# ade-ma/LibRedio

Measured on AMD Instinct MI355X. Metric: MSamples/s through FIR+FFT+resample chain, higher is better.
Workload: dtype f32

## Files before the change

libredio_amd/csrc/chain_v4.hip:

```cpp
#ifndef REDIO_EXP_CHAIN_NT
#define REDIO_EXP_CHAIN_NT 3
#endif
#include "fir_core.h"
#include "fft_wave.h"
#include "redio_internal.h"
#include "../../include/redio.h"
#include <type_traits>

namespace redio {

typedef float v4f_t __attribute__((ext_vector_type(4)));

template <int N, typename F>
__device__ __forceinline__ void static_for4(F &&f)
{
    if constexpr (N > 0) {
        static_for4<N - 1>(f);
        f(std::integral_constant<int, N - 1>{});
    }
}

template <int K, int D, bool FUSED, int WPS, int CH, bool FIR_ONLY, bool TWP, bool IN_U8, bool PF2, bool RES, int SCH>
__device__ __forceinline__ void chain_v4_body(const float2 *__restrict__ x, const float *__restrict__ taps,
                                              const float2 *__restrict__ tw, float2 *__restrict__ out,
                                              long nblocks, long blocks_per_wave, long wave, unsigned long long *dbg, long dbg_cap)
{
    unsigned long long t0c = 0, t0r = 0;
    if (dbg) { t0c = __builtin_amdgcn_s_memtime(); t0r = __builtin_amdgcn_s_memrealtime(); }
    constexpr int R = 4;
    using G = FirGeomV<K, D, R>;
    constexpr int SUB_OUT = 64 * R;
    constexpr int SUB_NEW = SUB_OUT * D;
    constexpr int HALO = G::tile_in(SUB_OUT) - SUB_NEW;
    static_assert(HALO % 2 == 0 && SUB_NEW % 128 == 0 && 4 * SUB_OUT == 1024, "geometry");
    constexpr int HALO_V = HALO / 2;
    constexpr int NLD = SUB_NEW / 2 / 64;
    static_assert(HALO_V <= 64, "the halo moves with one instruction per lane");
    extern __shared__ __attribute__((aligned(16))) char smem[];
    v4f_t *xs4 = reinterpret_cast<v4f_t *>(smem);
    float2 *ex = reinterpret_cast<float2 *>(smem);

    const int lane = threadIdx.x;
    const long b0 = wave * blocks_per_wave;
    if (b0 >= nblocks) return;
    const long b1 = (b0 + blocks_per_wave < nblocks) ? b0 + blocks_per_wave : nblocks;
    const long nsub = 4 * (b1 - b0);
    typename std::conditional<RES, FirTapsResident<K>, FirNoResidentTaps>::type rtaps;
    if constexpr (RES) fir_taps_resident_load(rtaps, taps);
    using pair_t = typename std::conditional<IN_U8, unsigned, v4f_t>::type;
    const pair_t *src0 = (IN_U8 ? reinterpret_cast<const pair_t *>(reinterpret_cast<const unsigned *>(x) + b0 * 512 * (long)D)
                                : reinterpret_cast<const pair_t *>(x + b0 * 1024 * (long)D)) + lane;
    auto samples = [](pair_t w) -> v4f_t {
        if constexpr (IN_U8) return v4f_t{i2f(w & 255u), i2f((w >> 8) & 255u), i2f((w >> 16) & 255u), i2f(w >> 24)};
        else return w;
    };

    pair_t pre[NLD], pre2[PF2 ? NLD : 1];
    __amdgpu_buffer_rsrc_t rs;
    if constexpr (PF2) {
        static_assert(!PF2 || !IN_U8, "PF2: cf32 input");
        rs = __builtin_amdgcn_make_buffer_rsrc(const_cast<float2 *>(x + b0 * 1024 * (long)D), 0, (int)((HALO + nsub * SUB_NEW) * 8), 0x00020000);
    }
    auto fetch_to = [&](pair_t(&dst)[NLD], long j) {
        if constexpr (PF2) {
            typedef unsigned v4u_t __attribute__((ext_vector_type(4)));
            const unsigned vo = 16u * (unsigned)lane + (unsigned)((HALO + j * SUB_NEW) * 8);
            static_for4<NLD>([&](auto I) {
                constexpr int k = I.value;
                const v4u_t w = __builtin_amdgcn_raw_buffer_load_b128(rs, vo + 1024u * (k & 3), 4096 * (k >> 2), 2 );
                dst[k] = __builtin_bit_cast(v4f_t, w);
            });
        } else {
            const pair_t *src = src0 + HALO_V + j * (SUB_NEW / 2);
#if REDIO_EXP_CHAIN_NT & 1
            static_for4<NLD>([&](auto I) { dst[I.value] = __builtin_nontemporal_load(src + 64 * I.value); });
#else
            static_for4<NLD>([&](auto I) { dst[I.value] = src[64 * I.value]; });
#endif
        }
    };
    auto park_from = [&](pair_t(&from)[NLD]) {
#if REDIO_EXP_ABLATE == 3
#pragma unroll
        for (int i = 0; i < NLD; ++i) { pair_t keep = from[i]; asm volatile("" : : "v"(keep)); }
#else
        static_for4<NLD>([&](auto I) { xs4[G::lds_index(HALO + 2 * (lane + 64 * I.value)) / 2] = samples(from[I.value]); });
#endif
    };

    if (lane < HALO_V) xs4[G::lds_index(2 * lane) / 2] = samples(src0[0]);
    static_assert(SCH == 0 || (!PF2 && !FIR_ONLY && TWP && WPS == 2), "the block schedules: the transforming product forms");
    constexpr int EXH_OFF = G::lds_elems(SUB_OUT) > FFT1KN_LDS ? G::lds_elems(SUB_OUT) : FFT1KN_LDS;
    constexpr int T12_OFF = EXH_OFF + (SCH == 2 ? FFT1KN_HALF_LDS : 0);
    static_assert(SCH == 0 || (T12_OFF + 60) * sizeof(float2) <= 160 * 1024 / 8 - 480, "within the request of chain_v4_lds at two waves per SIMD");
    if constexpr ((PF2 || SCH != 0) && !FIR_ONLY) {
        if (lane < 60) {
            const int k4 = lane / 15, i = lane % 15;
            const int idx = i < 3 ? 64 * k4 * (i + 1) : 16 * (k4 + 4 * ((i - 3) / 3)) * ((i - 3) % 3 + 1);
            ex[T12_OFF + lane] = tw[idx];
        }
    }
    fetch_to(pre, 0);
    park_from(pre);
    wave_lds_fence();

    float2 a[16];
#pragma unroll
    for (int i = 0; i < 16; ++i) a[i] = make_float2(0.f, 0.f);
    Fft1knTw34 t34;
    if (!FIR_ONLY && TWP) fft1kn_load_tw34(t34, lane, tw);
    auto step = [&](long j, auto ahead, auto place, pair_t(&req)[NLD], pair_t(&parked)[NLD]) {
        constexpr int AHEAD = decltype(ahead)::value, S = decltype(place)::value;
        const bool more = S >= 0 || j + 1 < nsub;
        if (S >= 0 || j + AHEAD < nsub) fetch_to(req, j + AHEAD);
        float2 acc[R];
#pragma unroll
        for (int r = 0; r < R; ++r) acc[r] = make_float2(0.f, 0.f);
        int lf = lane;
        asm volatile("" : "+v"(lf));
        if constexpr (RES) fir_lane_v_res<K, D, R, FUSED, CH>(xs4, lf, rtaps, acc);
        else fir_lane_v<K, D, R, FUSED, CH>(xs4, lf, taps, acc);
        if (FIR_ONLY) {
            v4f_t *y4 = reinterpret_cast<v4f_t *>(out + (b0 * 4 + j) * SUB_OUT) + 2 * lane;
            y4[0] = v4f_t{acc[0].x, acc[0].y, acc[1].x, acc[1].y};
            y4[1] = v4f_t{acc[2].x, acc[2].y, acc[3].x, acc[3].y};
        } else {
#pragma unroll
            for (int i = 0; i < 12; ++i) a[i] = a[i + 4];
#pragma unroll
            for (int r = 0; r < R; ++r) a[12 + r] = acc[r];
        }
        wave_lds_fence();
        v4f_t halo = v4f_t{0.f, 0.f, 0.f, 0.f};
        if (more && lf < HALO_V) halo = xs4[G::lds_index(SUB_NEW + 2 * lf) / 2];
        if (!FIR_ONLY && (S == 3 || (S < 0 && (j & 3) == 3))) {
            wave_lds_fence();
            int ln = lane;
            asm volatile("" : "+v"(ln));
            Fft1knTw12 t12;
            if constexpr (PF2) {
                const float2 *T = ex + T12_OFF + 15 * (ln >> 4);
#pragma unroll
                for (int i = 0; i < 3; ++i) t12.a[i] = T[i];
#pragma unroll
                for (int i = 0; i < 12; ++i) t12.b[i] = T[3 + i];
            } else fft1kn_load_tw12(t12, ln, tw);
            if (!TWP) fft1kn_load_tw34(t34, ln, tw);
            fft1kn_wave_tw<false>(a, ex, tw, t12, t34, out + (b0 + (j >> 2)) * 1024, ln);
            wave_lds_fence();
        }
        if (more) {
            if (lf < HALO_V) xs4[G::lds_index(2 * lf) / 2] = halo;
            park_from(parked);
        }
        wave_lds_fence();
    };
    [[maybe_unused]] float2 one = make_float2(0.f, 0.f);
    if constexpr (SCH != 0) {
        one = tw[0];
        asm volatile("" : "+v"(one.x), "+v"(one.y));
    }
    [[maybe_unused]] auto t12_lds = [&](Fft1knTw12 &t12, int ln) {
        const float2 *T = ex + T12_OFF + 15 * (ln >> 4);
#pragma unroll
        for (int i = 0; i < 3; ++i) t12.a[i] = T[i];
#pragma unroll
        for (int i = 0; i < 12; ++i) t12.b[i] = T[3 + i];
    };
    [[maybe_unused]] auto sstep = [&](long j, auto place, bool more_, bool xform_, auto &&hook) {
        constexpr int S = decltype(place)::value;
        const bool more = S < 3 || more_, xform = S == 3 && xform_;
        if (more) fetch_to(pre, j + 1);
        float2 acc[R];
#pragma unroll
        for (int r = 0; r < R; ++r) acc[r] = make_float2(0.f, 0.f);
        int lf = lane;
        asm volatile("" : "+v"(lf));
        if constexpr (RES) fir_lane_v_res<K, D, R, FUSED, CH>(xs4, lf, rtaps, acc, hook);
        else fir_lane_v<K, D, R, FUSED, CH>(xs4, lf, taps, acc, hook);
#pragma unroll
        for (int r = 0; r < R; ++r) a[4 * S + r] = acc[r];
        wave_lds_fence();
        v4f_t halo = v4f_t{0.f, 0.f, 0.f, 0.f};
        if (more && lf < HALO_V) halo = xs4[G::lds_index(SUB_NEW + 2 * lf) / 2];
        if (xform) {
            wave_lds_fence();
            int ln = lane;
            asm volatile("" : "+v"(ln));
            Fft1knTw12 t12;
            t12_lds(t12, ln);
            const float2 one1[1] = {one};
            fft1kn_wave_tw<false>(a, ex, one1, t12, t34, out + (b0 + (j >> 2)) * 1024, ln);
            wave_lds_fence();
        }
        if (more) {
            if (lf < HALO_V) xs4[G::lds_index(2 * lf) / 2] = halo;
            park_from(pre);
        }
        wave_lds_fence();
    };
    using S0 = std::integral_constant<int, 0>;
    using S1 = std::integral_constant<int, 1>;
    using S2 = std::integral_constant<int, 2>;
    using S3 = std::integral_constant<int, 3>;
    if constexpr (SCH == 1) {
        const long nb = b1 - b0;
#pragma unroll 1
        for (long blk = 0; blk < nb; ++blk) {
            sstep(4 * blk, S0{}, true, false, FirNoHook{});
            sstep(4 * blk + 1, S1{}, true, false, FirNoHook{});
            sstep(4 * blk + 2, S2{}, true, false, FirNoHook{});
            sstep(4 * blk + 3, S3{}, blk + 1 < nb, true, FirNoHook{});
        }
    } else if constexpr (SCH == 2) {
        constexpr int NCH = fir_num_chunks<K, D, R, CH>();
        const long nb = b1 - b0;
        sstep(0, S0{}, true, false, FirNoHook{});
#pragma unroll 1
        for (long blk = 0;; ++blk) {
            sstep(4 * blk + 1, S1{}, true, false, FirNoHook{});
            sstep(4 * blk + 2, S2{}, true, false, FirNoHook{});
            const bool more = blk + 1 < nb;
            sstep(4 * blk + 3, S3{}, more, !more, FirNoHook{});
            if (!more) break;
            float2 ap[16], u[16];
#pragma unroll
            for (int i = 0; i < 16; ++i) ap[i] = a[i];
            int ln = lane;
            asm volatile("" : "+v"(ln));
            Fft1knTw12 t12;
            float2 *dst = out + (b0 + blk) * 1024;
            auto piece = [&](auto C) {
                fft1kn_wave_piece<decltype(C)::value, false>(ap, u, ex + EXH_OFF, one, ex + T12_OFF + 15 * (ln >> 4), t12, t34, dst, ln);
            };
            sstep(4 * blk + 4, S0{}, true, false, piece);
            if constexpr (NCH < FFT1KN_PIECES)
                static_for4<FFT1KN_PIECES - NCH>([&](auto I) { piece(std::integral_constant<int, NCH + I.value>{}); });
        }
    } else if constexpr (PF2) {
        fetch_to(pre, 1);
        using two = std::integral_constant<int, 2>;
#pragma unroll 1
        for (long j = 0; j < nsub; j += 4) {
            step(j, two{}, std::integral_constant<int, 0>{}, pre2, pre);
            step(j + 1, two{}, std::integral_constant<int, 1>{}, pre, pre2);
            step(j + 2, two{}, std::integral_constant<int, 2>{}, pre2, pre);
            step(j + 3, two{}, std::integral_constant<int, 3>{}, pre, pre2);
        }
    } else {
#pragma unroll 1
        for (long j = 0; j < nsub; ++j) step(j, std::integral_constant<int, 1>{}, std::integral_constant<int, -1>{}, pre, pre);
    }
    if (dbg && lane == 0 && (long)blockIdx.x < dbg_cap) {
        dbg[4 * blockIdx.x] = __builtin_amdgcn_s_memtime() - t0c;
        dbg[4 * blockIdx.x + 1] = __builtin_amdgcn_s_memrealtime() - t0r;
        dbg[4 * blockIdx.x + 2] = t0r;
        unsigned xcc = 0;
        asm volatile("s_getreg_b32 %0, hwreg(HW_REG_XCC_ID)" : "=s"(xcc));
        unsigned hwid = 0;
        asm volatile("s_getreg_b32 %0, hwreg(HW_REG_HW_ID)" : "=s"(hwid));
        dbg[4 * blockIdx.x + 3] = ((unsigned long long)xcc << 32) | hwid;
    }
}

template <int WPS, bool FIR_ONLY, bool TWP, bool PF2, bool RES>
constexpr int chain_v4_sched()
{
    return (WPS == 2 && !FIR_ONLY && TWP && !PF2) ? 1 : 0;
}

template <int K, int D, bool FUSED, int WPS, int CH, bool FIR_ONLY = false, bool TWP = false, bool IN_U8 = false, bool PF2 = false>
__global__ __launch_bounds__(64, WPS) void chain_v4_kernel(const float2 *__restrict__ x, const float *__restrict__ taps,
                                                           const float2 *__restrict__ tw, float2 *__restrict__ out,
                                                           long nblocks, long blocks_per_wave, unsigned long long *dbg, long dbg_cap)
{
    chain_v4_body<K, D, FUSED, WPS, CH, FIR_ONLY, TWP, IN_U8, PF2, true, chain_v4_sched<WPS, FIR_ONLY, TWP, PF2, true>()>(x, taps, tw, out, nblocks, blocks_per_wave, (long)blockIdx.x, dbg, dbg_cap);
}
template <int K, int D, bool FUSED, int WPS, int CH, bool FIR_ONLY = false, bool TWP = false, bool IN_U8 = false, bool PF2 = false>
__global__ __launch_bounds__(64, WPS) void chain_v4_anytaps_kernel(const float2 *__restrict__ x, const float *__restrict__ taps,
                                                                   const float2 *__restrict__ tw, float2 *__restrict__ out,
                                                                   long nblocks, long blocks_per_wave, unsigned long long *dbg, long dbg_cap)
{
    chain_v4_body<K, D, FUSED, WPS, CH, FIR_ONLY, TWP, IN_U8, PF2, false, chain_v4_sched<WPS, FIR_ONLY, TWP, PF2, false>()>(x, taps, tw, out, nblocks, blocks_per_wave, (long)blockIdx.x, dbg, dbg_cap);
}

#ifdef REDIO_MEASURE
template <int K, int D, bool FUSED>
__global__ __launch_bounds__(64, 2) void chain_v4_sched2_kernel(const float2 *__restrict__ x, const float *__restrict__ taps,
                                                                const float2 *__restrict__ tw, float2 *__restrict__ out,
                                                                long nblocks, long blocks_per_wave, unsigned long long *dbg, long dbg_cap)
{
    chain_v4_body<K, D, FUSED, 2, 8, false, true, false, false, true, 2>(x, taps, tw, out, nblocks, blocks_per_wave, (long)blockIdx.x, dbg, dbg_cap);
}
#endif

struct ChainList {
    const float2 *x[REDIO_LIST_MAX];
    float2 *out[REDIO_LIST_MAX];
    long nblocks[REDIO_LIST_MAX];
    unsigned wave0[REDIO_LIST_MAX + 1];
    int count;
};

template <int K, int D, bool FUSED, bool RES>
__device__ __forceinline__ void chain_v4_list_body(const ChainList &list, const float *__restrict__ taps, const float2 *__restrict__ tw,
                                                   long blocks_per_wave)
{
    const unsigned w = blockIdx.x;
    int m = 0;
    for (int i = 1; i < list.count; ++i) m = w >= list.wave0[i] ? i : m;
    m = __builtin_amdgcn_readfirstlane(m);
    chain_v4_body<K, D, FUSED, 2, 8, false, true, false, false, RES, chain_v4_sched<2, false, true, false, RES>()>(list.x[m], taps, tw, list.out[m], list.nblocks[m], blocks_per_wave,
                                                                     (long)(w - list.wave0[m]), nullptr, 0);
}

template <int K, int D, bool FUSED>
__global__ __launch_bounds__(64, 2) void chain_v4_list_kernel(const ChainList list, const float *__restrict__ taps,
                                                              const float2 *__restrict__ tw, long blocks_per_wave)
{
    chain_v4_list_body<K, D, FUSED, true>(list, taps, tw, blocks_per_wave);
}
template <int K, int D, bool FUSED>
__global__ __launch_bounds__(64, 2) void chain_v4_anytaps_list_kernel(const ChainList list, const float *__restrict__ taps,
                                                                      const float2 *__restrict__ tw, long blocks_per_wave)
{
    chain_v4_list_body<K, D, FUSED, false>(list, taps, tw, blocks_per_wave);
}

long chain_v4_blocks_per_wave(long nblocks, int WPS)
{
    long waves = 4L * WPS * num_cus();
    if (waves > nblocks) waves = nblocks;
    if (waves < 1) waves = 1;
    long bpw = nblocks / (6 * waves);
    if (bpw < 1) bpw = 1;
    if (bpw > 4) bpw = 4;
    if (const char *e = measure_env("REDIO_CHAIN_BPW")) { const long v = atol(e); if (v >= 1) bpw = v; }
    return bpw;
}

template <int K, int D, int WPS, bool PF2 = false>
static constexpr size_t chain_v4_lds()
{
    static_assert(WPS == 2 || WPS == 3, "two wavefronts per SIMD (the chain: its transform needs 197 registers) or three (the FIR alone: 94-145)");
    using G = FirGeomV<K, D, 4>;
    constexpr int ELEMS = (G::lds_elems(256) > FFT1KN_LDS ? G::lds_elems(256) : FFT1KN_LDS) + (PF2 ? 64 : 0);
    constexpr size_t LDS_NEED = (size_t)ELEMS * sizeof(float2);
    static_assert(4 * WPS * LDS_NEED <= 160 * 1024, "4*WPS waves per CU");
    constexpr size_t LDS = (160 * 1024 / (4 * WPS)) - 480 > LDS_NEED ? (160 * 1024 / (4 * WPS)) - 480 : LDS_NEED;
    static_assert((4 * WPS + 1) * LDS > 160 * 1024, "one more wave must not fit");
    return LDS;
}

template <int K, int D, int WPS, int CH, bool FIR_ONLY = false, bool TWP = false, bool IN_U8 = false, bool PF2 = false>
static hipError_t launch_v4_t(const float2 *x, const float *taps, bool pal, const float2 *tw, float2 *out, long nblocks, bool fused,
                              hipStream_t s, unsigned long long *dbg, long dbg_cap = 0)
{
    constexpr size_t LDS = chain_v4_lds<K, D, WPS, PF2>();
    const long bpw = chain_v4_blocks_per_wave(nblocks, WPS);
    const long grid = (nblocks + bpw - 1) / bpw;
    if (pal) {
        if (fused) hipLaunchKernelGGL((chain_v4_kernel<K, D, true, WPS, CH, FIR_ONLY, TWP, IN_U8, PF2>), dim3((unsigned)grid), dim3(64), LDS, s, x, taps, tw, out, nblocks, bpw, dbg, dbg_cap);
        else hipLaunchKernelGGL((chain_v4_kernel<K, D, false, WPS, CH, FIR_ONLY, TWP, IN_U8, PF2>), dim3((unsigned)grid), dim3(64), LDS, s, x, taps, tw, out, nblocks, bpw, dbg, dbg_cap);
    } else {
        if (fused) hipLaunchKernelGGL((chain_v4_anytaps_kernel<K, D, true, WPS, CH, FIR_ONLY, TWP, IN_U8, PF2>), dim3((unsigned)grid), dim3(64), LDS, s, x, taps, tw, out, nblocks, bpw, dbg, dbg_cap);
        else hipLaunchKernelGGL((chain_v4_anytaps_kernel<K, D, false, WPS, CH, FIR_ONLY, TWP, IN_U8, PF2>), dim3((unsigned)grid), dim3(64), LDS, s, x, taps, tw, out, nblocks, bpw, dbg, dbg_cap);
    }
    return hipGetLastError();
// ... 106 lines not shown
```

libredio_amd/csrc/fft_wave.h:

```cpp
#pragma once
#include "fft_core.h"

namespace redio {

__device__ __forceinline__ void wave_lds_fence()
{
    __builtin_amdgcn_fence(__ATOMIC_RELEASE, "wavefront");
    __builtin_amdgcn_wave_barrier();
    __builtin_amdgcn_fence(__ATOMIC_ACQUIRE, "wavefront");
}

template <bool INV, typename TwPtr>
__device__ __forceinline__ void fft1k_wave_stages0to3(float2 (&v)[16], float2 *ex, TwPtr tw, const Fft1kTw &t, int lane)
{
    fft1k_passA<INV>(v, tw);
    wave_lds_fence();
#pragma unroll
    for (int k4 = 0; k4 < 4; ++k4)
#pragma unroll
        for (int k3 = 0; k3 < 4; ++k3) ex[fft1k_A_store(lane, k3, k4)] = v[k3 + 4 * k4];
    wave_lds_fence();
#pragma unroll
    for (int e = 0; e < 16; ++e) v[e] = ex[fft1k_B_load(lane, e)];
    wave_lds_fence();
    fft1k_passB<INV>(v, t);
#pragma unroll
    for (int k2 = 0; k2 < 4; ++k2)
#pragma unroll
        for (int k1 = 0; k1 < 4; ++k1) ex[fft1k_B_store(lane, k1, k2)] = v[k1 + 4 * k2];
    wave_lds_fence();
#pragma unroll
    for (int q = 0; q < 4; ++q)
#pragma unroll
        for (int j = 0; j < 4; ++j) v[4 * q + j] = ex[fft1k_C_load(lane, q, j)];
}

template <bool INV, typename DstPtr, typename TwPtr>
__device__ __forceinline__ void fft1k_wave_regs(float2 (&v)[16], DstPtr dst, float2 *ex, TwPtr tw, const Fft1kTw &t, int lane)
{
    fft1k_wave_stages0to3<INV>(v, ex, tw, t, lane);
    fft1k_passC<INV>(v, t);
#pragma unroll
    for (int q = 0; q < 4; ++q)
#pragma unroll
        for (int j = 0; j < 4; ++j) dst[lane + 64 * q + 256 * j] = v[4 * q + j];
}

template <bool INV, typename SrcPtr>
__device__ __forceinline__ void fft1k_wave(SrcPtr src, float2 *dst, float2 *ex,
                                           const float2 *__restrict__ tw, int lane)
{
    float2 v[16];
#pragma unroll
    for (int t = 0; t < 16; ++t) v[t] = src[lane + 64 * t];
    Fft1kTw t;
    fft1k_load_tw(t, lane, tw);
    fft1k_wave_regs<INV>(v, dst, ex, tw, t, lane);
}

}

namespace redio {

__device__ __forceinline__ void fft1kn_store_spectrum(const float2 (&a)[16], float2 *dst, int ln)
{
#pragma unroll
    for (int k0 = 0; k0 < 4; ++k0)
#pragma unroll
#if defined(REDIO_EXP_CHAIN_NT) && (REDIO_EXP_CHAIN_NT & 2)
        for (int k1 = 0; k1 < 4; ++k1) {
            typedef float nt_v2f __attribute__((ext_vector_type(2)));
            __builtin_nontemporal_store(nt_v2f{a[k1 + 4 * k0].x, a[k1 + 4 * k0].y}, reinterpret_cast<nt_v2f *>(dst + ln + 64 * k1 + 256 * k0));
        }
#else
        for (int k1 = 0; k1 < 4; ++k1) dst[ln + 64 * k1 + 256 * k0] = a[k1 + 4 * k0];
#endif
}

template <bool INV>
__device__ __forceinline__ void fft1kn_wave_tw(float2 (&a)[16], float2 *ex, const float2 *__restrict__ tw, const Fft1knTw12 &t12,
                                               const Fft1knTw34 &t34, float2 *dst, int ln)
{
    fft1kn_stage0<INV>(a, tw);
#pragma unroll
    for (int k4 = 0; k4 < 4; ++k4)
#pragma unroll
        for (int d0 = 0; d0 < 4; ++d0) ex[fft1kn_x1_store(ln, k4, d0)] = a[4 * k4 + d0];
    wave_lds_fence();
#pragma unroll
    for (int e = 0; e < 16; ++e) a[e] = ex[fft1kn_x1_load(ln, e)];
    wave_lds_fence();
    fft1kn_pass12<INV>(a, t12);
#pragma unroll
    for (int k3 = 0; k3 < 4; ++k3)
#pragma unroll
        for (int k2 = 0; k2 < 4; ++k2) ex[fft1kn_x2_store(ln, k2, k3)] = a[k2 + 4 * k3];
    wave_lds_fence();
#pragma unroll
    for (int f = 0; f < 16; ++f) a[f] = ex[fft1kn_x2_load(ln, f)];
    wave_lds_fence();
    fft1kn_pass34<INV>(a, t34);
    fft1kn_store_spectrum(a, dst, ln);
}

constexpr int FFT1KN_PIECES = 8;
template <int P, bool INV>
__device__ __forceinline__ void fft1kn_wave_piece(float2 (&a)[16], float2 (&u)[16], float2 *exh, float2 one, const float2 *T12, Fft1knTw12 &t12,
                                                  const Fft1knTw34 &t34, float2 *dst, int ln)
{
    if constexpr (P == 0) {
        const float2 one1[1] = {one};
        fft1kn_stage0<INV>(a, one1);
        if (fft1kn_x1h_store_half(ln) == 0) {
#pragma unroll
            for (int k4 = 0; k4 < 4; ++k4)
#pragma unroll
                for (int d0 = 0; d0 < 4; ++d0) exh[fft1kn_x1h_store(ln, k4, d0)] = a[4 * k4 + d0];
        }
    } else if constexpr (P == 1 || P == 2) {
        constexpr int h = P - 1;
        wave_lds_fence();
#pragma unroll
        for (int e = 8 * h; e < 8 * h + 8; ++e) u[e] = exh[fft1kn_x1h_load(ln, e)];
        wave_lds_fence();
        if constexpr (h == 0) {
            if (fft1kn_x1h_store_half(ln) == 1) {
#pragma unroll
                for (int k4 = 0; k4 < 4; ++k4)
#pragma unroll
                    for (int d0 = 0; d0 < 4; ++d0) exh[fft1kn_x1h_store(ln, k4, d0)] = a[4 * k4 + d0];
            }
        } else {
#pragma unroll
            for (int i = 0; i < 3; ++i) t12.a[i] = T12[i];
#pragma unroll
            for (int i = 0; i < 12; ++i) t12.b[i] = T12[3 + i];
        }
    } else if constexpr (P == 3) {
        fft1kn_pass12<INV>(u, t12);
        if (fft1kn_x2h_store_half(ln) == 0) {
#pragma unroll
            for (int k3 = 0; k3 < 4; ++k3)
#pragma unroll
                for (int k2 = 0; k2 < 4; ++k2) exh[fft1kn_x2h_store(ln, k2, k3)] = u[k2 + 4 * k3];
        }
    } else if constexpr (P == 4 || P == 5) {
        constexpr int h = P - 4;
        wave_lds_fence();
#pragma unroll
        for (int f = 0; f < 16; ++f)
            if (fft1kn_x2h_load_half(f) == h) a[f] = exh[fft1kn_x2h_load(ln, f)];
        wave_lds_fence();
        if constexpr (h == 0) {
            if (fft1kn_x2h_store_half(ln) == 1) {
#pragma unroll
                for (int k3 = 0; k3 < 4; ++k3)
#pragma unroll
                    for (int k2 = 0; k2 < 4; ++k2) exh[fft1kn_x2h_store(ln, k2, k3)] = u[k2 + 4 * k3];
            }
        }
    } else if constexpr (P == 6) {
        fft1kn_pass34<INV>(a, t34);
    } else if constexpr (P == 7) {
        fft1kn_store_spectrum(a, dst, ln);
    }
}

template <bool INV>
__device__ __forceinline__ void fft1kn_wave(float2 (&a)[16], float2 *ex, const float2 *__restrict__ tw, float2 *dst, int ln)
{
    Fft1knTw12 t12;
    Fft1knTw34 t34;
    fft1kn_load_tw12(t12, ln, tw);
    fft1kn_load_tw34(t34, ln, tw);
    fft1kn_wave_tw<INV>(a, ex, tw, t12, t34, dst, ln);
}

}
```

libredio_amd/csrc/fir_core.h:

```cpp
#pragma once
#include "redio_device.h"
#ifndef REDIO_EXP_ABLATE
#define REDIO_EXP_ABLATE 0
#endif
#include <type_traits>

namespace redio {

template <int K, int D, int R>
struct FirGeom {
    static constexpr int LSTR = R * D;
    static constexpr int SPAN = (R - 1) * D + K;
    static constexpr bool PAD = (LSTR % 2) == 0;
    RD_HD static constexpr int lds_index(int n) { return PAD ? n + n / LSTR : n; }
    RD_HD static constexpr int tile_in(int tile_out) { return (tile_out - 1) * D + K; }
    RD_HD static constexpr int lds_elems(int tile_out) { return lds_index(tile_in(tile_out) - 1) + 1; }
};

template <typename T, int K, int D, int R, bool FUSED, typename LdsPtr, typename TapPtr>
RD_HD void fir_lane(LdsPtr xs, int lane_slot, TapPtr h, T (&acc)[R])
{
    using G = FirGeom<K, D, R>;
    const int base = lane_slot * (G::LSTR + (G::PAD ? 1 : 0));
#pragma unroll
    for (int m = 0; m < G::SPAN; ++m) {
        const T xv = xs[base + G::lds_index(m)];
#pragma unroll
        for (int r = 0; r < R; ++r) {
            const int j = m - r * D;
            if (j >= 0 && j < K) acc[r] = mac<FUSED>(xv, h[j], acc[r]);
        }
    }
}

}

namespace redio {

template <int K, int D, int R>
struct FirGeomV {
    static constexpr int LSTR = R * D;
    static_assert(LSTR % 2 == 0, "16-byte windows need an even lane stride");
    static constexpr int SPAN = (R - 1) * D + K;
    static constexpr int PADN = ((LSTR / 2) % 2 == 1) ? 0 : 2;
    static constexpr int LANE_STRIDE = LSTR + PADN;
    RD_HD static constexpr int lds_index(int n) { return n + PADN * (n / LSTR); }
    RD_HD static constexpr int tile_in(int tile_out) { return (tile_out - 1) * D + K; }
    RD_HD static constexpr int lds_elems(int tile_out) { return (lds_index(tile_in(tile_out) - 1) + 2) & ~1; }
};

template <int N, typename F>
RD_HD void fir_static_for(F &&f)
{
    if constexpr (N > 0) {
        fir_static_for<N - 1>(f);
        f(std::integral_constant<int, N - 1>{});
    }
}

template <int K, int D, int R, int CH>
struct FirChunkTaps {
    static constexpr int NT = 2 * CH + (R - 1) * D;
    RD_HD static constexpr int lo(int c) { return 2 * CH * c - (R - 1) * D; }
};

struct FirNoHook {
    template <typename C>
    RD_HD void operator()(C) const {}
};
template <int K, int D, int R, int CH>
RD_HD constexpr int fir_num_chunks() { return ((FirGeomV<K, D, R>::SPAN + 1) / 2 + CH - 1) / CH; }

template <int c, int K, int D, int R, bool FUSED, int CH, typename Q, typename Lds4Ptr, typename TapPtr, typename Hook>
RD_HD void fir_chunks_v(Lds4Ptr xs4, int base4, TapPtr h, Q (&q)[2][CH],
                        float (&hb)[2][FirChunkTaps<K, D, R, CH>::NT], float2 (&acc)[R], Hook &hook)
{
    using G = FirGeomV<K, D, R>;
    using T = FirChunkTaps<K, D, R, CH>;
    constexpr int NRD = (G::SPAN + 1) / 2;
    constexpr int NCH = (NRD + CH - 1) / CH;
    if constexpr (c < NCH) {
        RD_PIN_SV(hb[c & 1][T::NT - 1], q[c & 1][0]);
        fir_static_for<CH>([&](auto I) {
            constexpr int i = (c + 1) * CH + I.value;
#if REDIO_EXP_ABLATE == 1
            if constexpr (i < NRD && (I.value & 1)) q[(c + 1) & 1][I.value] = q[(c + 1) & 1][I.value - 1];
            else
#endif
            if constexpr (i < NRD) q[(c + 1) & 1][I.value] = xs4[base4 + G::lds_index(2 * i) / 2];
        });
        fir_static_for<T::NT>([&](auto J) {
            constexpr int j = T::lo(c + 1) + J.value;
            if constexpr (c + 1 < NCH && j >= 0 && j < K) hb[(c + 1) & 1][J.value] = h[j];
        });
        hook(std::integral_constant<int, c>{});
        fir_static_for<CH>([&](auto I) {
            constexpr int m = 2 * (c * CH + I.value);
            if constexpr (m < G::SPAN) {
                const Q v = q[c & 1][I.value];
                const float2 x0 = make_float2(v.x, v.y), x1 = make_float2(v.z, v.w);
                fir_static_for<R>([&](auto RR) {
                    constexpr int r = RR.value;
#if REDIO_EXP_ABLATE == 2
                    if constexpr (r & 1) return;
#endif
                    constexpr int j0 = m - r * D, j1 = m + 1 - r * D;
                    if constexpr (j0 >= 0 && j0 < K) acc[r] = mac<FUSED>(x0, hb[c & 1][j0 - T::lo(c)], acc[r]);
                    if constexpr (j1 >= 0 && j1 < K && m + 1 < G::SPAN) acc[r] = mac<FUSED>(x1, hb[c & 1][j1 - T::lo(c)], acc[r]);
                });
            }
        });
#pragma unroll
        for (int r = 0; r < R; ++r) RD_PIN_F2(acc[r]);
        RD_SCHED_BARRIER();
        fir_chunks_v<c + 1, K, D, R, FUSED, CH>(xs4, base4, h, q, hb, acc, hook);
    }
}

template <int K, int D, int R, bool FUSED, int CH = 8 , typename Lds4Ptr, typename TapPtr, typename Hook>
RD_HD void fir_lane_v(Lds4Ptr xs4, int lane_slot, TapPtr h, float2 (&acc)[R], Hook &&hook)
{
    using G = FirGeomV<K, D, R>;
    using Q = typename std::remove_cv<typename std::remove_reference<decltype(xs4[0])>::type>::type;
    constexpr int NRD = (G::SPAN + 1) / 2;
    using T = FirChunkTaps<K, D, R, CH>;
    const int base4 = lane_slot * (G::LANE_STRIDE / 2);
    Q q[2][CH];
    float hb[2][T::NT];
    fir_static_for<T::NT>([&](auto J) {
        constexpr int j = T::lo(0) + J.value;
        hb[0][J.value] = (j >= 0 && j < K) ? h[j] : 0.0f;
        hb[1][J.value] = 0.0f;
    });
    fir_static_for<CH>([&](auto I) {
        constexpr int i = I.value;
        if constexpr (i < NRD) q[0][i] = xs4[base4 + G::lds_index(2 * i) / 2];
    });
    fir_chunks_v<0, K, D, R, FUSED, CH>(xs4, base4, h, q, hb, acc, hook);
}
template <int K, int D, int R, bool FUSED, int CH = 8, typename Lds4Ptr, typename TapPtr>
RD_HD void fir_lane_v(Lds4Ptr xs4, int lane_slot, TapPtr h, float2 (&acc)[R])
{
    fir_lane_v<K, D, R, FUSED, CH>(xs4, lane_slot, h, acc, FirNoHook{});
}

template <int K>
struct FirTapsResident {
    static constexpr int NE = (K + 1) / 2;
    static constexpr int NP = (NE + 1) / 2;
    static_assert(K >= 3, "a pair never reads past the taps");
    RD_HD static constexpr int elem(int j) { return j < K - 1 - j ? j : K - 1 - j; }
    unsigned long long p[NP];
};

struct FirNoResidentTaps {};

template <int K, typename TapPtr>
RD_HD void fir_taps_resident_load(FirTapsResident<K> &t, TapPtr h)
{
    fir_static_for<FirTapsResident<K>::NP>([&](auto I) {
        constexpr int i = I.value;
#if defined(__HIP_DEVICE_COMPILE__)
        typedef unsigned long long u64a __attribute__((may_alias));
        t.p[i] = reinterpret_cast<const u64a *>(&h[0])[i];
        asm volatile("" : "+s"(t.p[i]));
#else
        unsigned lo, hi;
        const float a = h[2 * i], b = h[2 * i + 1];
        __builtin_memcpy(&lo, &a, 4);
        __builtin_memcpy(&hi, &b, 4);
        t.p[i] = (unsigned long long)lo | ((unsigned long long)hi << 32);
#endif
    });
}

template <int K, int D, int R>
struct FirLive {
    RD_HD static constexpr int lo(int m) { return m - (K - 1) <= 0 ? 0 : (m - (K - 1) + D - 1) / D; }
    RD_HD static constexpr int hi(int m) { return m / D < R - 1 ? m / D : R - 1; }
};

#if defined(__HIP_DEVICE_COMPILE__)
typedef redio_v2f fir_acc_t;
#else
typedef float2 fir_acc_t;
#endif

template <int m0, int K, int D, int R, bool TWO >
struct FirReadPlan {
    using L = FirLive<K, D, R>;
    using T = FirTapsResident<K>;
#if REDIO_EXP_ABLATE == 2
    RD_HD static constexpr bool live(int k) { return !(k & 1) && (k < 4 || TWO) && (k & 3) >= L::lo(m0 + k / 4) && (k & 3) <= L::hi(m0 + k / 4) && (k & 3) < R; }
#else
    RD_HD static constexpr bool live(int k) { return (k < 4 || TWO) && (k & 3) >= L::lo(m0 + k / 4) && (k & 3) <= L::hi(m0 + k / 4) && (k & 3) < R; }
#endif
    RD_HD static constexpr int elem(int k) { return live(k) ? T::elem(m0 + k / 4 - (k & 3) * D) : 0; }
    RD_HD static constexpr int pair(int k) { return elem(k) / 2; }
    RD_HD static constexpr unsigned en() { unsigned v = 0; for (int k = 0; k < 8; ++k) v |= (live(k) ? 1u : 0u) << k; return v; }
    RD_HD static constexpr unsigned hi() { unsigned v = 0; for (int k = 0; k < 8; ++k) v |= (unsigned)(elem(k) & 1) << k; return v; }
    RD_HD static constexpr unsigned nop_fused()
    {
        unsigned v = 0;
        int prev = m0 == 0 ? 0 : L::hi(m0 - 1);
        for (int k = 0; k < 8; ++k)
            if (live(k)) { if ((k & 3) == prev) v |= 1u << k; prev = k & 3; }
        return v;
    }
    RD_HD static constexpr unsigned nop_exact()
    {
        unsigned v = 0;
        for (int i = 0; i < 2; ++i) {
            int n = 0;
            for (int r = 0; r < 4; ++r) n += live(4 * i + r) ? 1 : 0;
            if (n == 1) v |= 1u << i;
        }
        return v;
    }
};

#if defined(__HIP_DEVICE_COMPILE__)
#define RD_FMA_SLOT(k, r, i)                                                                                             \
    ".if (%[nb] >> " #k ") & 1\ns_nop 0\n.endif\n"                                                                      \
    ".if (%[en] >> " #k ") & 1\n.if (%[hi] >> " #k ") & 1\n"                                                            \
    "v_pk_fma_f32 %[a" #r "], %[x" #i "], %[t" #k "], %[a" #r "] op_sel:[0,1,0] op_sel_hi:[1,1,1]\n.else\n"               \
    "v_pk_fma_f32 %[a" #r "], %[x" #i "], %[t" #k "], %[a" #r "] op_sel:[0,0,0] op_sel_hi:[1,0,1]\n.endif\n.endif\n"
#define RD_MUL_SLOT(k, r, i)                                                                                             \
    ".if (%[en] >> " #k ") & 1\n.if (%[hi] >> " #k ") & 1\n"                                                            \
    "v_pk_mul_f32 %[d" #r "], %[x" #i "], %[t" #k "] op_sel:[0,1] op_sel_hi:[1,1]\n.else\n"                               \
    "v_pk_mul_f32 %[d" #r "], %[x" #i "], %[t" #k "] op_sel:[0,0] op_sel_hi:[1,0]\n.endif\n.endif\n"
#define RD_ADD_SLOT(k, r) ".if (%[en] >> " #k ") & 1\nv_pk_add_f32 %[a" #r "], %[a" #r "], %[d" #r "]\n.endif\n"
#define RD_ONE_NOP(i) ".if (%[nb] >> " #i ") & 1\ns_nop 0\n.endif\n"
template <int m0, int K, int D, int R, bool FUSED, bool TWO>
RD_D void fir_read_res(redio_v2f x0, redio_v2f x1, const FirTapsResident<K> &t, redio_v2f (&a)[R])
{
    static_assert(R == 4, "four accumulators per lane");
    using P = FirReadPlan<m0, K, D, R, TWO>;
    if constexpr (FUSED)
        asm volatile(RD_FMA_SLOT(0, 0, 0) RD_FMA_SLOT(1, 1, 0) RD_FMA_SLOT(2, 2, 0) RD_FMA_SLOT(3, 3, 0)
                     RD_FMA_SLOT(4, 0, 1) RD_FMA_SLOT(5, 1, 1) RD_FMA_SLOT(6, 2, 1) RD_FMA_SLOT(7, 3, 1)
                     : [a0] "+v"(a[0]), [a1] "+v"(a[1]), [a2] "+v"(a[2]), [a3] "+v"(a[3])
                     : [x0] "v"(x0), [x1] "v"(x1), [t0] "s"(t.p[P::pair(0)]), [t1] "s"(t.p[P::pair(1)]), [t2] "s"(t.p[P::pair(2)]),
                       [t3] "s"(t.p[P::pair(3)]), [t4] "s"(t.p[P::pair(4)]), [t5] "s"(t.p[P::pair(5)]), [t6] "s"(t.p[P::pair(6)]),
                       [t7] "s"(t.p[P::pair(7)]), [en] "i"(P::en()), [hi] "i"(P::hi()), [nb] "i"(P::nop_fused()));
    else {
        redio_v2f d0, d1, d2, d3;
        asm volatile(RD_MUL_SLOT(0, 0, 0) RD_MUL_SLOT(1, 1, 0) RD_MUL_SLOT(2, 2, 0) RD_MUL_SLOT(3, 3, 0) RD_ONE_NOP(0)
                     RD_ADD_SLOT(0, 0) RD_ADD_SLOT(1, 1) RD_ADD_SLOT(2, 2) RD_ADD_SLOT(3, 3)
                     RD_MUL_SLOT(4, 0, 1) RD_MUL_SLOT(5, 1, 1) RD_MUL_SLOT(6, 2, 1) RD_MUL_SLOT(7, 3, 1) RD_ONE_NOP(1)
                     RD_ADD_SLOT(4, 0) RD_ADD_SLOT(5, 1) RD_ADD_SLOT(6, 2) RD_ADD_SLOT(7, 3)
                     : [a0] "+v"(a[0]), [a1] "+v"(a[1]), [a2] "+v"(a[2]), [a3] "+v"(a[3]), [d0] "=&v"(d0), [d1] "=&v"(d1), [d2] "=&v"(d2),
                       [d3] "=&v"(d3)
                     : [x0] "v"(x0), [x1] "v"(x1), [t0] "s"(t.p[P::pair(0)]), [t1] "s"(t.p[P::pair(1)]), [t2] "s"(t.p[P::pair(2)]),
                       [t3] "s"(t.p[P::pair(3)]), [t4] "s"(t.p[P::pair(4)]), [t5] "s"(t.p[P::pair(5)]), [t6] "s"(t.p[P::pair(6)]),
                       [t7] "s"(t.p[P::pair(7)]), [en] "i"(P::en()), [hi] "i"(P::hi()), [nb] "i"(P::nop_exact()));
    }
}
#undef RD_FMA_SLOT
#undef RD_MUL_SLOT
#undef RD_ADD_SLOT
#undef RD_ONE_NOP
#else
template <int m0, int K, int D, int R, bool FUSED, bool TWO>
RD_HD void fir_read_res(float2 x0, float2 x1, const FirTapsResident<K> &t, float2 (&a)[R])
{
    using P = FirReadPlan<m0, K, D, R, TWO>;
    for (int k = 0; k < 8; ++k) {
        if (!P::live(k)) continue;
        const int el = P::elem(k);
        const unsigned w = (unsigned)(t.p[el / 2] >> (32 * (el & 1)));
        float h;
        __builtin_memcpy(&h, &w, 4);
        a[k & 3] = mac<FUSED>(k < 4 ? x0 : x1, h, a[k & 3]);
    }
}
#endif

template <int c, int K, int D, int R, bool FUSED, int CH, typename Q, typename Lds4Ptr, typename Hook>
RD_HD void fir_chunks_res(Lds4Ptr xs4, int base4, const FirTapsResident<K> &t, Q (&q)[2][CH], fir_acc_t (&acc)[R], Hook &hook)
{
    using G = FirGeomV<K, D, R>;
    constexpr int NRD = (G::SPAN + 1) / 2;
    constexpr int NCH = (NRD + CH - 1) / CH;
    if constexpr (c < NCH) {
        RD_PIN_V(q[c & 1][0]);
        fir_static_for<CH>([&](auto I) {
            constexpr int i = (c + 1) * CH + I.value;
#if REDIO_EXP_ABLATE == 1
            if constexpr (i < NRD && (I.value & 1)) q[(c + 1) & 1][I.value] = q[(c + 1) & 1][I.value - 1];
            else
#endif
            if constexpr (i < NRD) q[(c + 1) & 1][I.value] = xs4[base4 + G::lds_index(2 * i) / 2];
        });
        hook(std::integral_constant<int, c>{});
        fir_static_for<CH>([&](auto I) {
            constexpr int m = 2 * (c * CH + I.value);
            if constexpr (m < G::SPAN) {
                const Q v = q[c & 1][I.value];
#if defined(__HIP_DEVICE_COMPILE__)
                const fir_acc_t x0 = __builtin_shufflevector(v, v, 0, 1), x1 = __builtin_shufflevector(v, v, 2, 3);
#else
                const fir_acc_t x0 = make_float2(v.x, v.y), x1 = make_float2(v.z, v.w);
#endif
                fir_read_res<m, K, D, R, FUSED, (m + 1 < G::SPAN)>(x0, x1, t, acc);
            }
        });
        RD_SCHED_BARRIER();
        fir_chunks_res<c + 1, K, D, R, FUSED, CH>(xs4, base4, t, q, acc, hook);
    }
}

template <int K, int D, int R, bool FUSED, int CH = 8, typename Lds4Ptr, typename Hook>
RD_HD void fir_lane_v_res(Lds4Ptr xs4, int lane_slot, const FirTapsResident<K> &t, float2 (&acc)[R], Hook &&hook)
{
    using G = FirGeomV<K, D, R>;
    using Q = typename std::remove_cv<typename std::remove_reference<decltype(xs4[0])>::type>::type;
    constexpr int NRD = (G::SPAN + 1) / 2;
    const int base4 = lane_slot * (G::LANE_STRIDE / 2);
    Q q[2][CH];
    fir_static_for<CH>([&](auto I) {
        constexpr int i = I.value;
        if constexpr (i < NRD) q[0][i] = xs4[base4 + G::lds_index(2 * i) / 2];
    });
    fir_acc_t a[R];
#if defined(__HIP_DEVICE_COMPILE__)
#pragma unroll
// ... 57 lines not shown
```

Baseline: 529,700.

## Use buffer loads/stores, hoist LDS slot indices, and overlap prologue loads

Adds a REDIO_EXP_SEAM switch, defaulting to all options on. It routes input fetches and spectrum/FIR output stores through buffer resources with scalar offsets and nontemporal policy bits. LDS park and halo slot indices are hoisted out of the loop, and the halo read moves into the last FIR chunk hook. The prologue issues all global loads (halo head, first tile, twiddles, resident taps) before any LDS writes, so the latencies overlap. This aims to cut address arithmetic and serialized prologue latency, at the cost of more live registers and sched_barriers that constrain the compiler's scheduling.

```diff
diff --git a/libredio_amd/csrc/chain_v4.hip b/libredio_amd/csrc/chain_v4.hip
--- a/libredio_amd/csrc/chain_v4.hip
+++ b/libredio_amd/csrc/chain_v4.hip
@@ -1,5 +1,8 @@
 #ifndef REDIO_EXP_CHAIN_NT
 #define REDIO_EXP_CHAIN_NT 3
+#endif
+#ifndef REDIO_EXP_SEAM
+#define REDIO_EXP_SEAM 15
 #endif
 #include "fir_core.h"
 #include "fft_wave.h"
@@ -10,6 +13,8 @@
 namespace redio {
 
 typedef float v4f_t __attribute__((ext_vector_type(4)));
+
+constexpr int chain_gcd(int a, int b) { return b == 0 ? a : chain_gcd(b, a % b); }
 
 template <int N, typename F>
 __device__ __forceinline__ void static_for4(F &&f)
@@ -48,27 +53,57 @@
     typename std::conditional<RES, FirTapsResident<K>, FirNoResidentTaps>::type rtaps;
     if constexpr (RES) fir_taps_resident_load(rtaps, taps);
     using pair_t = typename std::conditional<IN_U8, unsigned, v4f_t>::type;
-    const pair_t *src0 = (IN_U8 ? reinterpret_cast<const pair_t *>(reinterpret_cast<const unsigned *>(x) + b0 * 512 * (long)D)
+    [[maybe_unused]] const pair_t *src0 = (IN_U8 ? reinterpret_cast<const pair_t *>(reinterpret_cast<const unsigned *>(x) + b0 * 512 * (long)D)
                                 : reinterpret_cast<const pair_t *>(x + b0 * 1024 * (long)D)) + lane;
     auto samples = [](pair_t w) -> v4f_t {
         if constexpr (IN_U8) return v4f_t{i2f(w & 255u), i2f((w >> 8) & 255u), i2f((w >> 16) & 255u), i2f(w >> 24)};
         else return w;
     };
 
+    constexpr bool HOIST = (REDIO_EXP_SEAM & 1) != 0, BUF = PF2 || (REDIO_EXP_SEAM & 2) != 0, EARLY = (REDIO_EXP_SEAM & 4) != 0,
+                   PRO = (REDIO_EXP_SEAM & 8) != 0;
+    auto slot = [](int p) { return G::lds_index(2 * p) / 2; };
+    constexpr int HSTR = G::LSTR / 2;
+    static_assert((SUB_NEW / 2) % HSTR == 0, "a sub-tile is a whole number of lane strides");
+    constexpr int HALO_DELTA = G::lds_index(SUB_NEW) / 2;
+    constexpr int PER0 = G::PADN == 0 ? 1 : HSTR / chain_gcd(64, HSTR), PER = PER0 < NLD ? PER0 : NLD;
+    constexpr int PARK_STEP = G::lds_index(2 * 64 * PER) / 2;
+    static_assert(PER == NLD || (64 * PER) % HSTR == 0, "park slots repeat with period PER");
+    auto halo_slots = [&](int lf, int &src, int &dst) {
+        dst = slot(lf);
+        if constexpr (EARLY) src = dst + (lf < HALO_V ? HALO_DELTA : 0);
+        else src = slot(SUB_NEW / 2 + lf);
+    };
+    [[maybe_unused]] int park4[PER], hsrc4 = 0, hdst4 = 0;
+    if constexpr (HOIST) {
+        static_for4<PER>([&](auto I) { park4[I.value] = slot(HALO_V + lane + 64 * I.value); });
+        halo_slots(lane, hsrc4, hdst4);
+    }
+
     pair_t pre[NLD], pre2[PF2 ? NLD : 1];
-    __amdgpu_buffer_rsrc_t rs;
-    if constexpr (PF2) {
+    constexpr unsigned PB = sizeof(pair_t);
+    constexpr int NT_LD = (REDIO_EXP_CHAIN_NT & 1) ? 2 : 0, NT_ST = (REDIO_EXP_CHAIN_NT & 2) ? 2 : 0;
+    typedef unsigned v4u_t __attribute__((ext_vector_type(4)));
+    typedef unsigned v2u_t __attribute__((ext_vector_type(2)));
+    [[maybe_unused]] __amdgpu_buffer_rsrc_t ri, ro;
+    if constexpr (BUF) {
         static_assert(!PF2 || !IN_U8, "PF2: cf32 input");
-        rs = __builtin_amdgcn_make_buffer_rsrc(const_cast<float2 *>(x + b0 * 1024 * (long)D), 0, (int)((HALO + nsub * SUB_NEW) * 8), 0x00020000);
-    }
+        const char *xb = reinterpret_cast<const char *>(x) + b0 * (512 * (long)D) * PB;
+        ri = __builtin_amdgcn_make_buffer_rsrc(const_cast<char *>(xb), 0, (int)((HALO_V + nsub * (SUB_NEW / 2)) * PB), 0x00020000);
+        ro = __builtin_amdgcn_make_buffer_rsrc(out + b0 * 1024, 0, (int)((b1 - b0) * 8192), 0x00020000);
+    }
+    [[maybe_unused]] auto buf_load = [&](unsigned vo, unsigned so, auto policy) -> pair_t {
+        if constexpr (IN_U8) return __builtin_amdgcn_raw_buffer_load_b32(ri, vo, so, decltype(policy)::value);
+        else return __builtin_bit_cast(v4f_t, __builtin_amdgcn_raw_buffer_load_b128(ri, vo, so, decltype(policy)::value));
+    };
     auto fetch_to = [&](pair_t(&dst)[NLD], long j) {
-        if constexpr (PF2) {
-            typedef unsigned v4u_t __attribute__((ext_vector_type(4)));
-            const unsigned vo = 16u * (unsigned)lane + (unsigned)((HALO + j * SUB_NEW) * 8);
+        if constexpr (BUF) {
+            const unsigned sub = (unsigned)((HALO_V + j * (SUB_NEW / 2)) * PB);
+            const unsigned vo = PB * (unsigned)lane + (PF2 ? sub : 0u), so = PF2 ? 0u : sub;
             static_for4<NLD>([&](auto I) {
-                constexpr int k = I.value;
-                const v4u_t w = __builtin_amdgcn_raw_buffer_load_b128(rs, vo + 1024u * (k & 3), 4096 * (k >> 2), 2 );
-                dst[k] = __builtin_bit_cast(v4f_t, w);
+                constexpr unsigned off = 64u * PB * I.value, imm = off % 4096u;
+                dst[I.value] = buf_load(vo + imm, so + (off - imm), std::integral_constant<int, NT_LD>{});
+                if constexpr (!PF2) __builtin_amdgcn_sched_barrier(0);
             });
         } else {
             const pair_t *src = src0 + HALO_V + j * (SUB_NEW / 2);
@@ -84,31 +119,99 @@
 #pragma unroll
         for (int i = 0; i < NLD; ++i) { pair_t keep = from[i]; asm volatile("" : : "v"(keep)); }
 #else
-        static_for4<NLD>([&](auto I) { xs4[G::lds_index(HALO + 2 * (lane + 64 * I.value)) / 2] = samples(from[I.value]); });
-#endif
-    };
-
-    if (lane < HALO_V) xs4[G::lds_index(2 * lane) / 2] = samples(src0[0]);
+        static_for4<NLD>([&](auto I) {
+            constexpr int i = I.value;
+            if constexpr (HOIST) xs4[park4[i % PER] + (i / PER) * PARK_STEP] = samples(from[i]);
+            else xs4[G::lds_index(HALO + 2 * (lane + 64 * i)) / 2] = samples(from[i]);
+        });
+#endif
+    };
+    [[maybe_unused]] auto store_block = [&](const float2(&a)[16], long blk, int ln) {
+        if constexpr (BUF) {
+            const unsigned so = (unsigned)(blk * 8192);
+            static_for4<16>([&](auto I) {
+                constexpr unsigned k0 = I.value / 4, k1 = I.value % 4;
+                const float2 v = a[k1 + 4 * k0];
+                __builtin_amdgcn_raw_buffer_store_b64(v2u_t{__builtin_bit_cast(unsigned, v.x), __builtin_bit_cast(unsigned, v.y)}, ro,
+                                                      8u * (unsigned)ln + (512u * k1 + 2048u * (k0 & 1)), so + 4096u * (k0 >> 1), NT_ST);
+            });
+        } else fft1kn_store_spectrum(a, out + (b0 + blk) * 1024, ln);
+    };
+
     static_assert(SCH == 0 || (!PF2 && !FIR_ONLY && TWP && WPS == 2), "the block schedules: the transforming product forms");
     constexpr int EXH_OFF = G::lds_elems(SUB_OUT) > FFT1KN_LDS ? G::lds_elems(SUB_OUT) : FFT1KN_LDS;
     constexpr int T12_OFF = EXH_OFF + (SCH == 2 ? FFT1KN_HALF_LDS : 0);
-    static_assert(SCH == 0 || (T12_OFF + 60) * sizeof(float2) <= 160 * 1024 / 8 - 480, "within the request of chain_v4_lds at two waves per SIMD");
-    if constexpr ((PF2 || SCH != 0) && !FIR_ONLY) {
-        if (lane < 60) {
-            const int k4 = lane / 15, i = lane % 15;
-            const int idx = i < 3 ? 64 * k4 * (i + 1) : 16 * (k4 + 4 * ((i - 3) / 3)) * ((i - 3) % 3 + 1);
-            ex[T12_OFF + lane] = tw[idx];
-        }
-    }
-    fetch_to(pre, 0);
-    park_from(pre);
-    wave_lds_fence();
+    constexpr bool TABLE = (PF2 || SCH != 0) && !FIR_ONLY;
+    static_assert(!TABLE || (T12_OFF + 64) * sizeof(float2) <= 160 * 1024 / 8 - 480, "within the request of chain_v4_lds at two waves per SIMD");
+    auto table_index = [](int l) {
+        const int k4 = l / 15, i = l % 15;
+        return i < 3 ? 64 * k4 * (i + 1) : 16 * (k4 + 4 * ((i - 3) / 3)) * ((i - 3) % 3 + 1);
+    };
+    Fft1knTw34 t34;
+    [[maybe_unused]] float2 one = make_float2(0.f, 0.f);
+    if constexpr (PRO) {
+        pair_t head;
+        if constexpr (BUF) head = buf_load(PB * (unsigned)lane, 0u, std::integral_constant<int, 0>{});
+        else head = src0[0];
+        fetch_to(pre, 0);
+        [[maybe_unused]] float2 twv = make_float2(0.f, 0.f);
+        if constexpr (TABLE) twv = tw[table_index(lane < 60 ? lane : 0)];
+        if (!FIR_ONLY && TWP) fft1kn_load_tw34(t34, lane, tw);
+        if constexpr (SCH != 0) one = tw[0];
+        xs4[slot(lane)] = samples(head);
+        if constexpr (TABLE) ex[T12_OFF + lane] = twv;
+        park_from(pre);
+        wave_lds_fence();
+    } else {
+        if (lane < HALO_V) {
+            if constexpr (BUF) xs4[slot(lane)] = samples(buf_load(PB * (unsigned)lane, 0u, std::integral_constant<int, 0>{}));
+            else xs4[slot(lane)] = samples(src0[0]);
+        }
+        if constexpr (TABLE)
+            if (lane < 60) ex[T12_OFF + lane] = tw[table_index(lane)];
+        fetch_to(pre, 0);
+        park_from(pre);
+        wave_lds_fence();
+        if (!FIR_ONLY && TWP) fft1kn_load_tw34(t34, lane, tw);
+        if constexpr (SCH != 0) one = tw[0];
+    }
+    if constexpr (SCH != 0) asm volatile("" : "+v"(one.x), "+v"(one.y));
 
     float2 a[16];
-#pragma unroll
-    for (int i = 0; i < 16; ++i) a[i] = make_float2(0.f, 0.f);
-    Fft1knTw34 t34;
-    if (!FIR_ONLY && TWP) fft1kn_load_tw34(t34, lane, tw);
+    if constexpr (!(PRO && SCH == 1)) {
+#pragma unroll
+        for (int i = 0; i < 16; ++i) a[i] = make_float2(0.f, 0.f);
+    }
+    constexpr int NCH = fir_num_chunks<K, D, R, CH>();
+    struct Seam { int lf, hs, hd; v4f_t halo; };
+    auto fir = [&](Seam &s, float2(&acc)[R], auto &&hook) {
+        s.lf = lane, s.hs = hsrc4, s.hd = hdst4, s.halo = v4f_t{0.f, 0.f, 0.f, 0.f};
+        if constexpr (!HOIST) {
+            asm volatile("" : "+v"(s.lf));
+            if constexpr (EARLY) halo_slots(s.lf, s.hs, s.hd);
+        }
+        auto hk = [&](auto C) {
+            if constexpr (EARLY && decltype(C)::value == NCH - 1) s.halo = xs4[s.hs];
+            hook(C);
+        };
+        if constexpr (RES) fir_lane_v_res<K, D, R, FUSED, CH>(xs4, s.lf, rtaps, acc, hk);
+        else fir_lane_v<K, D, R, FUSED, CH>(xs4, s.lf, taps, acc, hk);
+    };
+    auto halo_read = [&](Seam &s, bool more) {
+        if constexpr (!EARLY) {
+            if constexpr (!HOIST) halo_slots(s.lf, s.hs, s.hd);
+            if (more && s.lf < HALO_V) s.halo = xs4[s.hs];
+        }
+    };
+    auto halo_write = [&](const Seam &s) {
+        if constexpr (EARLY) xs4[s.hd] = s.halo;
+        else if (s.lf < HALO_V) xs4[HOIST ? s.hd : slot(s.lf)] = s.halo;
+    };
+    auto transform_lane = [&]() {
+        int ln = lane;
+        if constexpr (!HOIST) asm volatile("" : "+v"(ln));
+        return ln;
+    };
     auto step = [&](long j, auto ahead, auto place, pair_t(&req)[NLD], pair_t(&parked)[NLD]) {
         constexpr int AHEAD = decltype(ahead)::value, S = decltype(place)::value;
         const bool more = S >= 0 || j + 1 < nsub;
@@ -116,14 +219,19 @@
         float2 acc[R];
 #pragma unroll
         for (int r = 0; r < R; ++r) acc[r] = make_float2(0.f, 0.f);
-        int lf = lane;
-        asm volatile("" : "+v"(lf));
-        if constexpr (RES) fir_lane_v_res<K, D, R, FUSED, CH>(xs4, lf, rtaps, acc);
-        else fir_lane_v<K, D, R, FUSED, CH>(xs4, lf, taps, acc);
+        Seam seam;
+        fir(seam, acc, FirNoHook{});
         if (FIR_ONLY) {
-            v4f_t *y4 = reinterpret_cast<v4f_t *>(out + (b0 * 4 + j) * SUB_OUT) + 2 * lane;
-            y4[0] = v4f_t{acc[0].x, acc[0].y, acc[1].x, acc[1].y};
-            y4[1] = v4f_t{acc[2].x, acc[2].y, acc[3].x, acc[3].y};
+            const v4f_t y0 = v4f_t{acc[0].x, acc[0].y, acc[1].x, acc[1].y}, y1 = v4f_t{acc[2].x, acc[2].y, acc[3].x, acc[3].y};
+            if constexpr (BUF) {
+                const unsigned so = (unsigned)(j * (SUB_OUT * 8));
+                __builtin_amdgcn_raw_buffer_store_b128(__builtin_bit_cast(v4u_t, y0), ro, 32u * (unsigned)lane, so, 0);
+                __builtin_amdgcn_raw_buffer_store_b128(__builtin_bit_cast(v4u_t, y1), ro, 32u * (unsigned)lane + 16u, so, 0);
+            } else {
+                v4f_t *y4 = reinterpret_cast<v4f_t *>(out + (b0 * 4 + j) * SUB_OUT) + 2 * lane;
+                y4[0] = y0;
+                y4[1] = y1;
+            }
         } else {
 #pragma unroll
             for (int i = 0; i < 12; ++i) a[i] = a[i + 4];
@@ -131,12 +239,10 @@
             for (int r = 0; r < R; ++r) a[12 + r] = acc[r];
         }
         wave_lds_fence();
-        v4f_t halo = v4f_t{0.f, 0.f, 0.f, 0.f};
-        if (more && lf < HALO_V) halo = xs4[G::lds_index(SUB_NEW + 2 * lf) / 2];
+        halo_read(seam, more);
         if (!FIR_ONLY && (S == 3 || (S < 0 && (j & 3) == 3))) {
             wave_lds_fence();
-            int ln = lane;
-            asm volatile("" : "+v"(ln));
+            const int ln = transform_lane();
             Fft1knTw12 t12;
             if constexpr (PF2) {
                 const float2 *T = ex + T12_OFF + 15 * (ln >> 4);
@@ -146,20 +252,16 @@
                 for (int i = 0; i < 12; ++i) t12.b[i] = T[3 + i];
             } else fft1kn_load_tw12(t12, ln, tw);
             if (!TWP) fft1kn_load_tw34(t34, ln, tw);
-            fft1kn_wave_tw<false>(a, ex, tw, t12, t34, out + (b0 + (j >> 2)) * 1024, ln);
+            fft1kn_wave_regs<false>(a, ex, tw, t12, t34, ln);
+            store_block(a, j >> 2, ln);
             wave_lds_fence();
         }
         if (more) {
-            if (lf < HALO_V) xs4[G::lds_index(2 * lf) / 2] = halo;
+            halo_write(seam);
             park_from(parked);
         }
         wave_lds_fence();
     };
-    [[maybe_unused]] float2 one = make_float2(0.f, 0.f);
-    if constexpr (SCH != 0) {
-        one = tw[0];
-        asm volatile("" : "+v"(one.x), "+v"(one.y));
-    }
     [[maybe_unused]] auto t12_lds = [&](Fft1knTw12 &t12, int ln) {
         const float2 *T = ex + T12_OFF + 15 * (ln >> 4);
 #pragma unroll
@@ -174,27 +276,24 @@
         float2 acc[R];
 #pragma unroll
         for (int r = 0; r < R; ++r) acc[r] = make_float2(0.f, 0.f);
-        int lf = lane;
-        asm volatile("" : "+v"(lf));
-        if constexpr (RES) fir_lane_v_res<K, D, R, FUSED, CH>(xs4, lf, rtaps, acc, hook);
-        else fir_lane_v<K, D, R, FUSED, CH>(xs4, lf, taps, acc, hook);
+        Seam seam;
+        fir(seam, acc, hook);
 #pragma unroll
         for (int r = 0; r < R; ++r) a[4 * S + r] = acc[r];
         wave_lds_fence();
-        v4f_t halo = v4f_t{0.f, 0.f, 0.f, 0.f};
-        if (more && lf < HALO_V) halo = xs4[G::lds_index(SUB_NEW + 2 * lf) / 2];
+        halo_read(seam, more);
         if (xform) {
             wave_lds_fence();
-            int ln = lane;
-            asm volatile("" : "+v"(ln));
+            const int ln = transform_lane();
             Fft1knTw12 t12;
             t12_lds(t12, ln);
             const float2 one1[1] = {one};
-            fft1kn_wave_tw<false>(a, ex, one1, t12, t34, out + (b0 + (j >> 2)) * 1024, ln);
+            fft1kn_wave_regs<false>(a, ex, one1, t12, t34, ln);
+            store_block(a, j >> 2, ln);
             wave_lds_fence();
         }
         if (more) {
-            if (lf < HALO_V) xs4[G::lds_index(2 * lf) / 2] = halo;
+            halo_write(seam);
             park_from(pre);
         }
         wave_lds_fence();
@@ -213,7 +312,6 @@
             sstep(4 * blk + 3, S3{}, blk + 1 < nb, true, FirNoHook{});
         }
     } else if constexpr (SCH == 2) {
-        constexpr int NCH = fir_num_chunks<K, D, R, CH>();
         const long nb = b1 - b0;
         sstep(0, S0{}, true, false, FirNoHook{});
 #pragma unroll 1
diff --git a/libredio_amd/csrc/fft_wave.h b/libredio_amd/csrc/fft_wave.h
--- a/libredio_amd/csrc/fft_wave.h
+++ b/libredio_amd/csrc/fft_wave.h
@@ -78,8 +78,8 @@
 }
 
 template <bool INV>
-__device__ __forceinline__ void fft1kn_wave_tw(float2 (&a)[16], float2 *ex, const float2 *__restrict__ tw, const Fft1knTw12 &t12,
-                                               const Fft1knTw34 &t34, float2 *dst, int ln)
+__device__ __forceinline__ void fft1kn_wave_regs(float2 (&a)[16], float2 *ex, const float2 *__restrict__ tw, const Fft1knTw12 &t12,
+                                                 const Fft1knTw34 &t34, int ln)
 {
     fft1kn_stage0<INV>(a, tw);
 #pragma unroll
@@ -100,6 +100,12 @@
     for (int f = 0; f < 16; ++f) a[f] = ex[fft1kn_x2_load(ln, f)];
     wave_lds_fence();
     fft1kn_pass34<INV>(a, t34);
+}
+template <bool INV>
+__device__ __forceinline__ void fft1kn_wave_tw(float2 (&a)[16], float2 *ex, const float2 *__restrict__ tw, const Fft1knTw12 &t12,
+                                               const Fft1knTw34 &t34, float2 *dst, int ln)
+{
+    fft1kn_wave_regs<INV>(a, ex, tw, t12, t34, ln);
     fft1kn_store_spectrum(a, dst, ln);
 }
 
diff --git a/libredio_amd/csrc/fir_core.h b/libredio_amd/csrc/fir_core.h
--- a/libredio_amd/csrc/fir_core.h
+++ b/libredio_amd/csrc/fir_core.h
@@ -158,6 +158,14 @@
 template <int K, typename TapPtr>
 RD_HD void fir_taps_resident_load(FirTapsResident<K> &t, TapPtr h)
 {
+#if defined(__HIP_DEVICE_COMPILE__) && !(defined(REDIO_EXP_SEAM) && !(REDIO_EXP_SEAM & 8))
+    fir_static_for<FirTapsResident<K>::NP>([&](auto I) {
+        typedef unsigned long long u64a __attribute__((may_alias));
+        t.p[I.value] = reinterpret_cast<const u64a *>(&h[0])[I.value];
+    });
+#pragma unroll
+    for (int i = 0; i < FirTapsResident<K>::NP; ++i) asm volatile("" : "+s"(t.p[i]));
+#else
     fir_static_for<FirTapsResident<K>::NP>([&](auto I) {
         constexpr int i = I.value;
 #if defined(__HIP_DEVICE_COMPILE__)
@@ -172,6 +180,7 @@
         t.p[i] = (unsigned long long)lo | ((unsigned long long)hi << 32);
 #endif
     });
+#endif
 }
 
 template <int K, int D, int R>
```

After: 536,300, median of 6. 1.3% higher.
